# Rafae1130/qwen_inference_engine

Measured on AMD Instinct MI355X. Metric: decode tokens/s + prefill tok/s, Qwen2-7B bf16 batch=1, 1/2/4/8 MI355X, higher is better.
Workload: dtype bf16; 1 GPU; Qwen2-7B bf16 decode, batch=1, prompt=2048, gen=512; batch_per_gpu=1, batch=1, prompt=2048, gen=512, parallelism=single, graph=True, kv=contiguous

## Files before the change

__graft_entry__.py:

```python
import os
import subprocess
import sys

ROOT = os.path.dirname(os.path.abspath(__file__))


def build() -> None:
    jobs = str(min(16, os.cpu_count() or 8))
    subprocess.check_call(["make", "-s", "-j", jobs, "-C", os.path.join(ROOT, "qwen_inference_engine_amd", "csrc")])
    subprocess.check_call(["make", "-s", "-C", os.path.join(ROOT, "oracle")])
    if os.path.isdir("/root/reference/layers/src"):
        subprocess.check_call(["make", "-s", "-C", os.path.join(ROOT, "oracle"), "ref"])
    sys.path.insert(0, ROOT)
    import qwen_inference_engine_amd as q
    from qwen_inference_engine_amd import _lib
    _lib.load()


def smoke() -> None:
    sys.path.insert(0, ROOT)
    sys.path.insert(0, os.path.join(ROOT, "oracle"))
    import numpy as np
    import oracle as O
    import qwen_inference_engine_amd as q
# ... 19 lines not shown
```

include/qie/qie_ops.h:

```cpp
#ifndef QIE_OPS_H
#define QIE_OPS_H

#include "qie_types.h"

#ifdef __cplusplus
extern "C" {
#endif

#define QIE_ABI_VERSION 1

const char* qie_last_error(void);
int qie_abi_version(void);
int qie_device_count(int* count);

int qie_set_device(int device);
int qie_malloc(void** ptr, int64_t bytes);
int qie_free(void* ptr);
int qie_memcpy_h2d(void* dst, const void* src, int64_t bytes);
int qie_memcpy_d2h(void* dst, const void* src, int64_t bytes);
int qie_memset(void* ptr, int value, int64_t bytes);
int qie_synchronize(void);
int qie_stream_create(void** stream_out);
int qie_stream_synchronize(void* stream);
int qie_stream_destroy(void* stream);
// ... 52 lines not shown
                 int32_t layer, float eps, int32_t numerics, void* q_out, void* stream);

int64_t qie_attention_workspace_bytes(int64_t M, int32_t n_heads, int32_t head_dim,
                                      int32_t max_ctx);
int qie_attention(const void* q, int64_t M, const int32_t* pos, int32_t rows_per_seq,
                  const qie_kv_cache* cache, int32_t layer, int32_t n_heads, void* out,
                  void* ws, void* stream);

int64_t qie_attention_extend_workspace_bytes(int64_t M, int32_t n_heads, int32_t head_dim,
                                             int32_t max_ctx);
int32_t qie_attention_extend_split_tokens(int64_t M, int32_t max_ctx);
int qie_attention_extend(const void* q, int64_t M, const int32_t* pos, int32_t rows_per_seq,
                         const qie_kv_cache* cache, int32_t layer, int32_t n_heads, void* out,
                         void* ws, void* stream);

#define QIE_NUMERICS_MASK 0xff
#define QIE_ATTN_PREROPED 0x100
int64_t qie_attention_decode_workspace_bytes(int64_t B, int32_t n_heads, int32_t n_kv_heads,
                                             int32_t head_dim, int32_t max_ctx);
int qie_attention_decode(const void* qkv, int64_t B, const int32_t* pos, const void* q_norm,
                         const void* k_norm, const float* rope_cos, const float* rope_sin,
                         int32_t n_heads, const qie_kv_cache* cache, int32_t layer, float eps,
                         int32_t numerics, void* out, void* ws, void* stream);

int qie_debug_tr16_probe(int32_t* out_dev);

int qie_qknorm(void* x, int64_t rows, int64_t row_stride, int32_t n_heads, int32_t head_dim,
               const void* w, float eps, int32_t numerics, void* stream);
int qie_rope(void* x, int64_t rows, int64_t row_stride, int32_t n_heads, int32_t head_dim,
             const int32_t* pos, int32_t pos0, const float* rope_cos, const float* rope_sin,
// ... 57 lines not shown
```

qwen_inference_engine_amd/_lib.py:

```python
from __future__ import annotations

import ctypes as C
import os

_HERE = os.path.dirname(os.path.abspath(__file__))
LIB_PATH = os.environ.get("QIE_LIB") or os.path.join(_HERE, "lib", "libqie.so")

QIE_NUMERICS_REF = 0
QIE_NUMERICS_HF = 1
QIE_EPI_STORE = 0
QIE_EPI_RESIDUAL = 1
QIE_EPI_SWIGLU = 2
QIE_EPI_F32 = 3
QIE_LINEAR_FP8 = 1
QIE_LINEAR_TILE256 = 2
QIE_LINEAR_TILE128 = 4
QIE_LINEAR_STREAMK = 8
QIE_LINEAR_FP8_T16 = 16
QIE_LINEAR_ACT_FP8 = 32
QIE_ATTN_PREROPED = 0x100
QIE_VERIFY_MAX_ROWS = 16
QIE_SCORE_UNFUSED = 1
QIE_COMM_ID_BYTES = 128
QIE_COMM_PEER_HANDLE_BYTES = 128
# ... 70 lines not shown
    ("qie_stream_create", C.c_int, [C.POINTER(_P)]),
    ("qie_stream_synchronize", C.c_int, [_P]),
    ("qie_stream_destroy", C.c_int, [_P]),
    ("qie_rope_table_host", C.c_int, [_PF, _PF, _I32, _I32, _F, _I32]),
    ("qie_embedding", C.c_int, [_P, _P, _P, _I64, _I64, _P]),
    ("qie_rmsnorm", C.c_int, [_P, _P, _P, _I64, _I64, _F, _I32, _P]),
    ("qie_linear", C.c_int, [C.POINTER(LinearArgsC), _P]),
    ("qie_debug_linear_plan", C.c_int, [C.POINTER(LinearArgsC), C.c_char_p, C.c_int]),
    ("qie_qkv_post", C.c_int, [_P, _I64, _P, _I32, _P, _P, _P, _P, _I32, C.POINTER(KvCacheC),
                               _I32, _F, _I32, _P, _P]),
    ("qie_attention_workspace_bytes", C.c_int64, [_I64, _I32, _I32, _I32]),
    ("qie_attention", C.c_int, [_P, _I64, _P, _I32, C.POINTER(KvCacheC), _I32, _I32, _P, _P, _P]),
    ("qie_attention_extend_workspace_bytes", C.c_int64, [_I64, _I32, _I32, _I32]),
    ("qie_attention_extend_split_tokens", C.c_int32, [_I64, _I32]),
    ("qie_attention_extend", C.c_int, [_P, _I64, _P, _I32, C.POINTER(KvCacheC), _I32, _I32, _P, _P, _P]),
    ("qie_attention_decode_workspace_bytes", C.c_int64, [_I64, _I32, _I32, _I32, _I32]),
    ("qie_attention_decode", C.c_int, [_P, _I64, _P, _P, _P, _P, _P, _I32, C.POINTER(KvCacheC), _I32, _F, _I32,
                                       _P, _P, _P]),
    ("qie_debug_tr16_probe", C.c_int, [_P]),
    ("qie_qknorm", C.c_int, [_P, _I64, _I64, _I32, _I32, _P, _F, _I32, _P]),
    ("qie_rope", C.c_int, [_P, _I64, _I64, _I32, _I32, _P, _I32, _P, _P, _I32, _P]),
    ("qie_kv_write", C.c_int, [_P, _P, _I64, _I64, _I32, C.POINTER(KvCacheC), _I32, _I32, _P]),
    ("qie_kv_copy", C.c_int, [C.POINTER(KvCacheC), _I32, C.POINTER(KvCacheC), _I32, _I32, _I32, _P]),
    ("qie_silu", C.c_int, [_P, _I64, _P]),
    ("qie_mul", C.c_int, [_P, _P, _P, _I64, _P]),
    ("qie_memcpy_d2d", C.c_int, [_P, _P, _I64, _P]),
    ("qie_silu_mul", C.c_int, [_P, _P, _P, _I64, _P]),
    ("qie_residual_add", C.c_int, [_P, _P, _I64, _P]),
    ("qie_residual_add_f32", C.c_int, [_P, _P, _I64, _P]),
    ("qie_sample_workspace_bytes", C.c_int64, [_I64, _I64]),
# ... 113 lines not shown
```

qwen_inference_engine_amd/csrc/attn_mfma_tile.hpp:

```cpp
#pragma once
#include "attn_decode.hpp"

#include <type_traits>

namespace qie {

template <int HD, bool PG, int NW, bool SPLIT>
__device__ __forceinline__ void attn_mfma_walk(const uint16_t* kb, const uint16_t* vb, const KvMap& km, const int seq,
                                               const int kmax, const int k0, const int nkt,
                                               const bf16x8_t (&qf)[2][HD / 32], const int (&qpos)[2],
                                               const int (&gpos)[2], const int (&gmin)[2], f32x4_t (&oacc)[2][HD / 16],
                                               float (&m_run)[2], float (&l_run)[2]) {
    constexpr int KT = 64;
    constexpr int CPR = HD / 8;
    constexpr int KSTEPS = HD / 32;
    constexpr int DT = HD / 16;
    constexpr int QG = 2;
    extern __shared__ __attribute__((aligned(16))) unsigned char smem[];
    uint16_t* Ks = reinterpret_cast<uint16_t*>(smem);
    uint16_t* Vs = reinterpret_cast<uint16_t*>(smem + 2 * KT * HD * 2);
    auto vswz = [](int r) { return 2 * (r & (CPR / 2 - 1)); };

    const int tid = threadIdx.x, lane = tid & 63, wave = __builtin_amdgcn_readfirstlane(tid >> 6);
    const int fr = lane & 15, g = lane >> 4;
// ... 57 lines not shown
#pragma unroll
            for (int q = 0; q < QG; q++) {
                if (!ON[q]) continue;
                float (&sv)[4][4] = pv[q];
                float mt = -INFINITY;
                if (kt * KT + KT - 1 <= gmin[q]) {
#pragma unroll
                    for (int t = 0; t < 4; t++)
#pragma unroll
                        for (int r = 0; r < 4; r++) {
                            const float sc = sacc[q][t][r] * sl2;
                            sv[t][r] = sc;
                            mt = fmaxf(mt, sc);
                        }
                } else {
#pragma unroll
                    for (int t = 0; t < 4; t++)
#pragma unroll
                        for (int r = 0; r < 4; r++) {
                            const int key = kt * KT + t * 16 + g * 4 + r;
                            const float sc = key <= qpos[q] ? sacc[q][t][r] * sl2 : -INFINITY;
                            sv[t][r] = sc;
                            mt = fmaxf(mt, sc);
                        }
                }
                mt = xor32_max(xor16_max(mt));
                const float m_new = fmaxf(m_run[q], mt);
                const float m_use = SPLIT && m_new == -INFINITY ? 0.f : m_new;
                const float alpha = __builtin_amdgcn_exp2f(m_run[q] - m_use);
                float ls = 0.f;
#pragma unroll
                for (int t = 0; t < 4; t++)
#pragma unroll
                    for (int r = 0; r < 4; r++) {
                        const float e = __builtin_amdgcn_exp2f(sv[t][r] - m_use);
                        sv[t][r] = e;
// ... 99 lines not shown
```

qwen_inference_engine_amd/csrc/engine.hip:

```cpp
#include "qie_common.hpp"
#include "linear_plan.hpp"
#include "../../include/qie/qie_engine.h"
#include "qie_index.hpp"
#include "qie_comm.hpp"
#include "verify.hpp"
#include "row_bufs.hpp"
#include "page_pool.hpp"

#include <chrono>
#include <cstring>
#include <fstream>
#include <functional>
#include <vector>

namespace qie {
bool dec8_applies(const qie_linear_args* a);
int dec8_reserve(hipStream_t st);
bool persist_supported(const qie_model_spec& s, int B, int tp, bool fp8, bool paged, int ncu, const char** why);
size_t persist_attn_table_bytes(int n_layers);
int persist_attn_table(const qie_model_spec& s, const qie_layer_weights* h_layers, const void* qkv_scratch,
                       const int32_t* pos, const float* rope_cos, const float* rope_sin, const qie_kv_cache* cache,
                       void* dec_ws, void* d_attp, hipStream_t st);
int persist_decode_launch(const qie_model_spec& s, const qie_layer_weights* d_layers, const void* d_attp,
                          uint16_t* x_res, unsigned long long* granules, const unsigned* epoch, unsigned* err,
// ... 567 lines not shown

static int enqueue_layer_decode(qie_batch* b, int l) {
    qie_engine* e = b->e;
    const LayerPath p = decode_path(e);
    const qie_layer_weights& L = p.layers[l];
    const LayerRows r = layer_rows(b->dec, b->B, 1);
    QIE_TRY(run_proj(b, qkv_args(e, L, p.flags, r), p.in, r, decode_qkv_extras(b)));
    QIE_TRY(attend_decode(b, l, r.att));
    QIE_TRY(run_row_proj(b, o_args(e, L, p.flags, r), p.in, r));
    QIE_TRY(dbg_snap(b, 2 * l + 1));
    QIE_TRY(run_proj(b, gate_up_args(e, L, p.flags, r), p.in, r));
    QIE_TRY(run_row_proj(b, down_args(e, L, p.flags, r), p.in, r));
    return dbg_snap(b, 2 * l + 2);
}

using AttentionFn = decltype(&qie_attention);
static int enqueue_layer_rows(qie_batch* b, int l, const LayerRows& r, const LayerPath& p, const qie_kv_cache& cache,
                              AttentionFn attend, void* attn_ws) {
    qie_engine* e = b->e;
    const qie_model_spec& s = e->spec;
    const qie_layer_weights& L = p.layers[l];
    hipStream_t st = e->stream;
    QIE_TRY(run_proj(b, qkv_args(e, L, p.flags, r), p.in, r));
    QIE_TRY(qie_qkv_post(r.qkv, r.M, r.pos, r.rows_per_seq, L.q_norm, L.k_norm, e->rope_cos, e->rope_sin, e->sh.nq,
                         &cache, l, s.rms_eps, s.numerics, r.q, st));
    QIE_TRY(attend(r.q, r.M, r.pos, r.rows_per_seq, &cache, l, e->sh.nq, r.att, attn_ws, st));
    QIE_TRY(run_row_proj(b, o_args(e, L, p.flags, r), p.in, r));
    QIE_TRY(run_proj(b, gate_up_args(e, L, p.flags, r), p.in, r));
    return run_row_proj(b, down_args(e, L, p.flags, r), p.in, r);
}

static bool is_greedy(const qie_sampling* s) { return !s || s->top_k <= 1 || !(s->temperature > 0.f); }

__global__ void unshard_rows_kernel(const uint16_t* __restrict__ tmp, uint16_t* __restrict__ full, int tp, int M,
                                    int64_t Vl, int64_t V, int m0) {
    const int64_t n = (int64_t)tp * M * Vl;
    for (int64_t k = blockIdx.x * 256 + threadIdx.x; k < n; k += (int64_t)gridDim.x * 256) {
        const int64_t j = k % Vl, i = (k / Vl) % M, r = k / (Vl * M);
        full[(m0 + i) * V + r * Vl + j] = tmp[k];
    }
}
// ... 731 lines not shown
    }
    QIE_TRY(flush_table(b));
    const int64_t H = s.hidden;
    QIE_HIP(hipMemcpyAsync(b->pf.ids_in, ids, (size_t)n * 4, hipMemcpyHostToDevice, st));
    hipLaunchKernelGGL(iota_kernel, dim3((unsigned)((n + 255) / 256)), dim3(256), 0, st, b->pf.pos, (int)n, len, pos0);
    hipLaunchKernelGGL(copy_ids_kernel, dim3((len + 255) / 256, n_seqs), dim3(256), 0, st, b->pf.ids_in,
                       b->dec.hist + (int64_t)seq0 * b->max_ctx + pos0, len, (int64_t)b->max_ctx);
    QIE_TRY(qie_embedding(e->w.embed, b->pf.ids_in, b->pf.x, n, H, st));
    const qie_kv_cache cache = batch_cache(b, seq0);
    const LayerRows r = layer_rows(b->pf, n, len);
    const bool pf16 = e->fp8 && !e->layers_pf.empty() && (n >= 256 || (e->fp8_t16 && n > 16));
    LayerPath path{e->layers.data(), proj_flags(e), prefill_mx(e) ? InputForm::Fp8 : InputForm::Normed};
    if (pf16 && path.in == InputForm::Normed)
        path = LayerPath{e->layers_pf.data(), path.flags & ~(QIE_LINEAR_FP8 | QIE_LINEAR_FP8_T16), InputForm::Normed};
    for (int l = 0; l < s.n_layers; l++)
        QIE_TRY(enqueue_layer_rows(b, l, r, path, cache, append ? qie_attention_extend : qie_attention, b->pf_ws.p));
    for (int z = 0; z < n_seqs; z++) {
        hipLaunchKernelGGL(set_state_kernel, dim3(1), dim3(64), 0, st, seq0 + z, pos0 + len - 1, 0,
                           ids[(int64_t)z * len + len - 1], b->dec.pos, b->dec.step, b->dec.hist, b->max_ctx,
                           (const uint4*)e->w.embed, (uint4*)b->dec.x, (int64_t)H / 8, 0, rope_cur_args(b));
        QIE_LAUNCH_CHECK();
    }
    const uint16_t* last = b->pf.x + (int64_t)(len - 1) * H;
    if (n_seqs > 1) {
        QIE_HIP(hipMemcpy2DAsync(b->pf.xn, (size_t)H * 2, last, (size_t)len * H * 2, (size_t)H * 2, n_seqs,
                                 hipMemcpyDeviceToDevice, st));
        last = b->pf.xn;
    }
    QIE_TRY(enqueue_head(b, last, H, seq0, n_seqs, smp));
    for (int z = 0; z < n_seqs; z++) b->h_pos[seq0 + z] = pos0 + len;
    if (score) QIE_TRY(enqueue_score(b, seq0, len, *score));
// ... 358 lines not shown
    b->v = v;
    return 0;
}

static int enqueue_verify(qie_batch* b, int seq, int M, const qie_sampling* smp) {
    qie_engine* e = b->e;
    const qie_model_spec& s = e->spec;
    hipStream_t st = e->stream;
    const int64_t H8 = (int64_t)s.hidden / 8;
    VerifyRowsArgs ra{seq, M, b->v.draft, s.vocab, (const uint4*)e->w.embed, (const uint4*)b->dec.x, H8,
                      b->dec.pos, b->dec.step, (uint4*)b->v.x, b->v.pos, b->v.step};
    QIE_TRY(launch_verify_rows(ra, st));
    const qie_kv_cache cache = batch_cache(b, seq);
    const LayerRows r = layer_rows(b->v, M, M);
    for (int l = 0; l < s.n_layers; l++)
        QIE_TRY(enqueue_layer_rows(b, l, r, decode_path(e), cache, qie_attention_extend, b->v.attn_ws));
    QIE_TRY(enqueue_head_rows(b, b->v.x, s.hidden, M, smp, head_bufs(b->v, 0, b->e->sh.vocab)));
    const bool greedy = is_greedy(smp);
    VerifyCommitArgs ca{seq, M, greedy ? b->v.keys : nullptr, b->v.ids, b->v.draft, s.vocab, b->dec.pos, b->dec.step,
                        b->dec.hist, b->max_ctx, b->dec.ids, (const uint4*)e->w.embed, (uint4*)b->dec.x, H8,
                        rope_cur_args(b), b->v.logits, b->dec.logits, (int64_t)e->sh.vocab, b->v.res};
    return launch_verify_commit(ca, st);
}

static int launch_verify(qie_batch* b, int seq, int M, const qie_sampling* smp) {
    qie_engine* e = b->e;
    if (!e->opts.use_graph) return enqueue_verify(b, seq, M, smp);
    const bool greedy = is_greedy(smp);
    for (const auto& g : b->v_graphs)
        if (g.seq == seq && g.M == M && g.greedy == greedy && (greedy || same_sampling(g.smp, smp))) {
            QIE_HIP(hipGraphLaunch(g.exec, e->stream));
// ... 311 lines not shown
```

qwen_inference_engine_amd/csrc/k_attention.hip:

```cpp
#include "qie_common.hpp"
#include "../../include/qie/qie_ops.h"
#include "attn_mfma_tile.hpp"


#include <cstdlib>
#include <type_traits>

namespace qie {

struct AttnParams {
    const uint16_t* q;
    const int32_t* pos;
    int rows_per_seq;
    const uint16_t* kc;
    const uint16_t* vc;
    KvMap km;
    int layer, nkv, nq, max_ctx;
    int nsplit;
    float* part_o;
    float* part_ml;
    uint16_t* out;
};

template <int HD, bool PG>
__global__ __launch_bounds__(256) void attn_split_kernel(AttnParams a) {
    constexpr int LPT = HD / 8;
// ... 2 lines not shown
    __shared__ float sm_m[4][kMaxGroup], sm_l[4][kMaxGroup];

    const int64_t m = blockIdx.y;
    const int g = blockIdx.x / a.nsplit, s = blockIdx.x % a.nsplit;
    const int G = a.nq / a.nkv;
    const int lane = threadIdx.x & 63, wave = threadIdx.x >> 6;
    const int sub = lane / LPT, dl = lane % LPT;
    const int ctx = a.pos[m] + 1;
    int chunk = (ctx + a.nsplit - 1) / a.nsplit;
    chunk = (chunk + 4 * TPW - 1) / (4 * TPW) * (4 * TPW);
    const int t0 = s * chunk;
    const int t1 = min(ctx, t0 + chunk);
    const int64_t seq = m / a.rows_per_seq;

    float qf[kMaxGroup][8];
    const uint16_t* qrow = a.q + m * (int64_t)a.nq * HD + (int64_t)g * G * HD + dl * 8;
#pragma unroll
    for (int gi = 0; gi < kMaxGroup; gi++) {
        if (gi < G) {
            uint4 v = *reinterpret_cast<const uint4*>(qrow + gi * HD);
            uint32_t w[4] = {v.x, v.y, v.z, v.w};
#pragma unroll
            for (int j = 0; j < 4; j++) {
                qf[gi][2 * j] = bf_lo(w[j]);
                qf[gi][2 * j + 1] = bf_hi(w[j]);
            }
        } else {
#pragma unroll
            for (int j = 0; j < 8; j++) qf[gi][j] = 0.f;
        }
    }
    float mr[kMaxGroup], lr[kMaxGroup], o[kMaxGroup][8];
#pragma unroll
    for (int gi = 0; gi < kMaxGroup; gi++) {
        mr[gi] = -INFINITY;
// ... 88 lines not shown
        if (a.nsplit == 1) {
            a.out[m * (int64_t)a.nq * HD + (int64_t)h * HD + d] = f2bf(ov / l);
        } else {
            const int64_t pi = (m * a.nq + h) * (int64_t)a.nsplit + s;
            a.part_o[pi * HD + d] = ov;
            if (d == 0) {
                a.part_ml[pi * 2] = mn;
                a.part_ml[pi * 2 + 1] = l;
            }
        }
    }
}


struct PrefillAttnParams {
    const uint16_t* q;
    const int32_t* pos;
    int rows_per_seq;
    const uint16_t* kc;
    const uint16_t* vc;
    KvMap km;
    int layer, nkv, nq;
    uint16_t* out;
    int full_tiles;
};


template <int HD, bool PG, int NW>
__global__ __launch_bounds__(64 * NW, 8 / NW) void attn_prefill_mfma2_kernel(PrefillAttnParams a) {
    constexpr int KT = 64;
    constexpr int KSTEPS = HD / 32;
// ... 15 lines not shown
    bool gact[QG];
    gact[0] = j < npair;
    gact[1] = j < npair && grp[1] != j;
    const int kmax = a.pos[row0 + min(16 * (ngr - 1 - (int)blockIdx.x * NW) + 15, R - 1)];
    const int nkt = kmax / KT + 1;

    int qpos[QG], gpos[QG], gmin[QG];
    bf16x8_t qf[QG][KSTEPS];
#pragma unroll
    for (int q = 0; q < QG; q++) {
        const int gq = gact[q] ? grp[q] : 0;
        const int qrow = min(16 * gq + fr, R - 1);
        qpos[q] = a.pos[row0 + qrow];
        gpos[q] = __builtin_amdgcn_readfirstlane(gact[q] ? a.pos[row0 + min(16 * gq + 15, R - 1)] : -1);
        gmin[q] = __builtin_amdgcn_readfirstlane(a.full_tiles ? a.pos[row0 + min(16 * gq, R - 1)] : -1);
        const uint16_t* qp = a.q + (row0 + qrow) * (int64_t)a.nq * HD + (int64_t)h * HD;
#pragma unroll
        for (int ks = 0; ks < KSTEPS; ks++) qf[q][ks] = *reinterpret_cast<const bf16x8_t*>(qp + ks * 32 + g * 8);
    }

    f32x4_t oacc[QG][DT];
    float m_run[QG], l_run[QG];
    attn_mfma_walk<HD, PG, NW, false>(kb, vb, a.km, seq, kmax, 0, nkt, qf, qpos, gpos, gmin, oacc, m_run, l_run);
#pragma unroll
    for (int q = 0; q < QG; q++) {
        if (!gact[q]) continue;
        float lr[4];
#pragma unroll
        for (int r = 0; r < 4; r++) lr[r] = __shfl(l_run[q], g * 4 + r, 64);
#pragma unroll
        for (int r = 0; r < 4; r++) {
            const int row = 16 * grp[q] + g * 4 + r;
            if (row >= R) continue;
// ... 84 lines not shown
                           out, ws);
}

}

using namespace qie;

extern "C" {

int64_t qie_attention_workspace_bytes(int64_t M, int32_t n_heads, int32_t head_dim, int32_t max_ctx) {
    const int ns = attn_nsplit(M, max_ctx);
    if (ns == 1) return 0;
    return M * n_heads * (int64_t)ns * (head_dim + 2) * 4;
}

int qie_attention(const void* q, int64_t M, const int32_t* pos, int32_t rows_per_seq,
                  const qie_kv_cache* cache, int32_t layer, int32_t n_heads, void* out, void* ws,
                  void* stream) {
    QIE_REQUIRE(q && pos && cache && cache->k && cache->v && out && M >= 0 && rows_per_seq > 0,
                "qie_attention: bad arguments");
    QIE_REQUIRE(cache->head_dim == 64 || cache->head_dim == 128,
                "qie_attention: head_dim must be 64 or 128 (got %d)", cache->head_dim);
    QIE_REQUIRE(n_heads % cache->n_kv_heads == 0 && n_heads / cache->n_kv_heads <= kMaxGroup,
                "qie_attention: n_heads/n_kv_heads must be an integer <= %d", kMaxGroup);
    QIE_REQUIRE(layer >= 0 && layer < cache->n_layers, "qie_attention: bad layer");
    if (M == 0) return 0;
    if (rows_per_seq >= 32 && M % rows_per_seq == 0) {
        PrefillAttnParams pa;
        pa.q = (const uint16_t*)q;
        pa.pos = pos;
        pa.rows_per_seq = rows_per_seq;
        pa.kc = (const uint16_t*)cache->k;
        pa.vc = (const uint16_t*)cache->v;
        QIE_TRY(kv_map_make(cache, &pa.km, "qie_attention"));
        pa.layer = layer;
        pa.nkv = cache->n_kv_heads;
        pa.nq = n_heads;
        pa.out = (uint16_t*)out;
        pa.full_tiles = dev_env("QIE_ATTN_PF_FULL", 1);
        const size_t shm = (size_t)2 * 2 * 64 * cache->head_dim * 2;
        const bool pg = pa.km.table != nullptr;
        const int npair = ((rows_per_seq + 15) / 16 + 1) / 2;
        const int nw = dev_env("QIE_ATTN_PF_NW", 8) == 4 ? 4 : 8;
        dim3 g2((unsigned)((npair + nw - 1) / nw), (unsigned)n_heads, (unsigned)(M / rows_per_seq));
        auto k2 = nw == 8 ? (cache->head_dim == 128 ? (pg ? attn_prefill_mfma2_kernel<128, true, 8> : attn_prefill_mfma2_kernel<128, false, 8>)
                                                    : (pg ? attn_prefill_mfma2_kernel<64, true, 8> : attn_prefill_mfma2_kernel<64, false, 8>))
                          : (cache->head_dim == 128 ? (pg ? attn_prefill_mfma2_kernel<128, true, 4> : attn_prefill_mfma2_kernel<128, false, 4>)
                                                    : (pg ? attn_prefill_mfma2_kernel<64, true, 4> : attn_prefill_mfma2_kernel<64, false, 4>));
        hipLaunchKernelGGL(k2, g2, dim3(64 * nw), shm, (hipStream_t)stream, pa);
        QIE_LAUNCH_CHECK();
        return 0;
    }
    AttnParams a;
    a.q = (const uint16_t*)q;
    a.pos = pos;
    a.rows_per_seq = rows_per_seq;
    a.kc = (const uint16_t*)cache->k;
    a.vc = (const uint16_t*)cache->v;
    QIE_TRY(kv_map_make(cache, &a.km, "qie_attention"));
    a.layer = layer;
    a.nkv = cache->n_kv_heads;
    a.nq = n_heads;
    a.max_ctx = cache->max_ctx;
    a.nsplit = attn_nsplit(M, cache->max_ctx);
    const int64_t part = M * n_heads * (int64_t)a.nsplit;
    a.part_o = (float*)ws;
    a.part_ml = ws ? (float*)ws + part * cache->head_dim : nullptr;
    a.out = (uint16_t*)out;
    QIE_REQUIRE(a.nsplit == 1 || ws, "qie_attention: workspace required");
    hipStream_t st = (hipStream_t)stream;
    dim3 grid((unsigned)(a.nkv * a.nsplit), (unsigned)M);
    const bool pg = a.km.table != nullptr;
    auto k = cache->head_dim == 128 ? (pg ? attn_split_kernel<128, true> : attn_split_kernel<128, false>)
                                    : (pg ? attn_split_kernel<64, true> : attn_split_kernel<64, false>);
    hipLaunchKernelGGL(k, grid, dim3(256), 0, st, a);
    QIE_LAUNCH_CHECK();
    if (a.nsplit > 1) {
        launch_attn_combine<false>(cache->head_dim, M, n_heads, a.nsplit, a.part_o, a.part_ml, a.out, st);
        QIE_LAUNCH_CHECK();
    }
    return 0;
}

int qie_debug_tr16_probe(int32_t* out_dev) {
    QIE_REQUIRE(out_dev, "qie_debug_tr16_probe: null");
    hipLaunchKernelGGL(tr16_probe_kernel, dim3(1), dim3(64), 0, nullptr, out_dev);
    QIE_LAUNCH_CHECK();
    return 0;
}

int64_t qie_attention_decode_workspace_bytes(int64_t B, int32_t n_heads, int32_t n_kv_heads, int32_t head_dim,
                                             int32_t max_ctx) {
    const int64_t ns = std::min<int64_t>(kDecMaxSplits, (max_ctx + 63) / 64);
    const int64_t cnt = ((B * n_kv_heads * 4 + 255) / 256) * 256;
    return cnt + B * n_heads * ns * (head_dim + 2) * 4;
}
// ... 37 lines not shown
```

qwen_inference_engine_amd/csrc/k_attn_extend.hip:

```cpp
#include "qie_common.hpp"
#include "../../include/qie/qie_ops.h"
#include "attn_mfma_tile.hpp"

namespace qie {

constexpr int kExtSplitLong = 512;
constexpr int kExtSplitShort = 256;
constexpr int kExtShortRows = 32;
constexpr int kExtMaxSplits = 64;
constexpr int kExtBlockRows = 128;

static void extend_split(int64_t M, int32_t max_ctx, int* len, int* count) {
    int L = M <= kExtShortRows ? kExtSplitShort : kExtSplitLong;
    int n = (max_ctx + L - 1) / L;
    while (n > kExtMaxSplits) {
        L *= 2;
        n = (max_ctx + L - 1) / L;
    }
    *len = L;
    *count = n < 1 ? 1 : n;
}

struct ExtendAttnParams {
    const uint16_t* q;
    const int32_t* pos;
    int rows_per_seq;
    int64_t M;
    const uint16_t* kc;
    const uint16_t* vc;
    KvMap km;
    int layer, nkv, nq;
    int nsplit, split_len;
    float* part_o;
    float* part_ml;
    uint16_t* out;
};

template <int HD, bool PG>
__global__ __launch_bounds__(256, 2) void attn_extend_kernel(ExtendAttnParams a) {
// ... 35 lines not shown
    const uint16_t* vb = a.vc + head_off;

    const int grp[QG] = {wave, NGB - 1 - wave};
    bool gact[QG];
    int qpos[QG], gpos[QG], gmin[QG];
    bf16x8_t qf[QG][KSTEPS];
#pragma unroll
    for (int q = 0; q < QG; q++) {
        gact[q] = f0 + 16 * grp[q] < RG;
        const int fb = gact[q] ? f0 + 16 * grp[q] : f0;
        const int f = min(fb + fr, RG - 1);
        const int t = f / G, hq = f - t * G;
        qpos[q] = a.pos[row0 + t];
        gpos[q] = __builtin_amdgcn_readfirstlane(gact[q] ? a.pos[row0 + min(fb + 15, RG - 1) / G] : -1);
        gmin[q] = __builtin_amdgcn_readfirstlane(a.pos[row0 + fb / G]);
        const uint16_t* qp = a.q + (row0 + t) * (int64_t)a.nq * HD + (int64_t)(kvh * G + hq) * HD;
#pragma unroll
        for (int ks = 0; ks < KSTEPS; ks++) qf[q][ks] = *reinterpret_cast<const bf16x8_t*>(qp + ks * 32 + g * 8);
    }

    f32x4_t oacc[QG][DT];
    float m_run[QG], l_run[QG];
    attn_mfma_walk<HD, PG, NW, true>(kb, vb, a.km, seq, kmax, k0, nkt, qf, qpos, gpos, gmin, oacc, m_run, l_run);

#pragma unroll
    for (int q = 0; q < QG; q++) {
        if (!gact[q]) continue;
        const int fb = f0 + 16 * grp[q];
        if (a.nsplit == 1) {
            float lr[4];
#pragma unroll
            for (int r = 0; r < 4; r++) lr[r] = __shfl(l_run[q], g * 4 + r, 64);
#pragma unroll
// ... 29 lines not shown
extern "C" {

int32_t qie_attention_extend_split_tokens(int64_t M, int32_t max_ctx) {
    int len, count;
    extend_split(M, max_ctx, &len, &count);
    return len;
}

int64_t qie_attention_extend_workspace_bytes(int64_t M, int32_t n_heads, int32_t head_dim, int32_t max_ctx) {
    int len, count;
    extend_split(M, max_ctx, &len, &count);
    if (count == 1) return 0;
    return M * n_heads * (int64_t)count * (head_dim + 2) * 4;
}

int qie_attention_extend(const void* q, int64_t M, const int32_t* pos, int32_t rows_per_seq,
                         const qie_kv_cache* cache, int32_t layer, int32_t n_heads, void* out, void* ws,
                         void* stream) {
    QIE_REQUIRE(q && pos && cache && cache->k && cache->v && out && M >= 0 && rows_per_seq > 0 && n_heads > 0,
                "qie_attention_extend: bad arguments");
    QIE_REQUIRE(cache->head_dim == 64 || cache->head_dim == 128,
                "qie_attention_extend: head_dim must be 64 or 128 (got %d)", cache->head_dim);
    QIE_REQUIRE(cache->n_kv_heads > 0 && n_heads % cache->n_kv_heads == 0 &&
                    n_heads / cache->n_kv_heads <= kMaxGroup,
                "qie_attention_extend: n_heads/n_kv_heads must be an integer <= %d", kMaxGroup);
    QIE_REQUIRE(layer >= 0 && layer < cache->n_layers, "qie_attention_extend: bad layer");
    if (M == 0) return 0;
    ExtendAttnParams a;
    a.q = (const uint16_t*)q;
    a.pos = pos;
    a.rows_per_seq = rows_per_seq;
    a.M = M;
    a.kc = (const uint16_t*)cache->k;
    a.vc = (const uint16_t*)cache->v;
    QIE_TRY(kv_map_make(cache, &a.km, "qie_attention_extend"));
    a.layer = layer;
    a.nkv = cache->n_kv_heads;
    a.nq = n_heads;
    extend_split(M, cache->max_ctx, &a.split_len, &a.nsplit);
    QIE_REQUIRE(a.nsplit == 1 || ws, "qie_attention_extend: workspace required");
    const int64_t part = M * n_heads * (int64_t)a.nsplit;
    a.part_o = (float*)ws;
    a.part_ml = ws ? (float*)ws + part * cache->head_dim : nullptr;
    a.out = (uint16_t*)out;
// ... 5 lines not shown
    hipStream_t st = (hipStream_t)stream;
    const size_t shm = (size_t)2 * 2 * 64 * cache->head_dim * 2;
    const bool pg = a.km.table != nullptr;
    dim3 grid((unsigned)nblk, (unsigned)a.nsplit, (unsigned)(n_seqs * a.nkv));
    auto k = cache->head_dim == 128 ? (pg ? attn_extend_kernel<128, true> : attn_extend_kernel<128, false>)
                                    : (pg ? attn_extend_kernel<64, true> : attn_extend_kernel<64, false>);
    hipLaunchKernelGGL(k, grid, dim3(256), shm, st, a);
    QIE_LAUNCH_CHECK();
    if (a.nsplit > 1) {
        launch_attn_combine<true>(cache->head_dim, M, n_heads, a.nsplit, a.part_o, a.part_ml, a.out, st);
        QIE_LAUNCH_CHECK();
    }
    return 0;
}

}
```

qwen_inference_engine_amd/csrc/k_misc.hip:

```cpp
#include "qie_common.hpp"
#include "launch_util.hpp"
#include "../../include/qie/qie_ops.h"

#include <cmath>
#include <cstdarg>
#include <cstring>
#include <map>
#include <mutex>
#include <tuple>
#include <vector>

#ifdef _OPENMP
#include <omp.h>
#endif

namespace qie {

static thread_local std::string g_last_error;

void set_error(const std::string& msg) { g_last_error = msg; }

int fail(int code, const char* fmt, ...) {
    char buf[1024];
    va_list ap;
// ... 196 lines not shown
            float x0 = active ? bf2f((uint16_t)(raw[b] & 0xffffu)) : 0.f;
            float x1 = active ? bf2f((uint16_t)(raw[b] >> 16)) : 0.f;
            if (rope && nw) {
                float ss = wave_sum(x0 * x0 + x1 * x1);
                float rms = sqrtf((ss / (float)hd) + a.eps);
                if (HF) {
                    float inv = 1.0f / rms;
                    x0 = rbf(bf2f(nw[i0]) * rbf(x0 * inv));
                    x1 = rbf(bf2f(nw[i1]) * rbf(x1 * inv));
                } else {
                    x0 = rbf((x0 / rms) * bf2f(nw[i0]));
                    x1 = rbf((x1 / rms) * bf2f(nw[i1]));
                }
            }
            float y0 = x0, y1 = x1;
            if (rope) {
                if (HF) {
                    y0 = rbf(rbf(x0 * c) + rbf(-x1 * s));
                    y1 = rbf(rbf(x1 * c) + rbf(x0 * s));
                } else {
                    y0 = x0 * c - x1 * s;
                    y1 = x1 * c + x0 * s;
                }
            }
            if (active) {
                if (HF) {
                    dst[i0] = f2bf(y0);
                    dst[i1] = f2bf(y1);
                } else {
                    reinterpret_cast<uint32_t*>(dst)[lane] = pack2(y0, y1);
                }
            }
        }
    }
}

struct HeadOpArgs {
    uint16_t* x;
    int64_t row_stride;
    int nheads, hd;
    const uint16_t* w;
    float eps;
    const float* cs;
    const float* sn;
    const int32_t* pos;
    int pos0;
    int numerics;
    int rope;
};
// ... 404 lines not shown
    a.kc = (uint16_t*)cache->k;
    a.vc = (uint16_t*)cache->v;
    QIE_TRY(kv_map_make(cache, &a.km, "qie_qkv_post"));
    a.layer = layer;
    a.eps = eps;
    a.numerics = numerics;
    a.q_out = (uint16_t*)q_out;
    const bool hf = numerics == QIE_NUMERICS_HF;
    auto fn = a.km.table ? (hf ? qkv_post_kernel<true, true> : qkv_post_kernel<true, false>)
                         : (hf ? qkv_post_kernel<false, true> : qkv_post_kernel<false, false>);
    hipLaunchKernelGGL(fn, dim3((unsigned)M), dim3(256), 0, (hipStream_t)stream, a);
    QIE_LAUNCH_CHECK();
    return 0;
}

int qie_memcpy_d2d(void* dst, const void* src, int64_t bytes, void* stream) {
    QIE_REQUIRE(dst && src && bytes >= 0, "qie_memcpy_d2d: bad arguments");
    if (bytes == 0) return 0;
    QIE_HIP(hipMemcpyAsync(dst, src, (size_t)bytes, hipMemcpyDeviceToDevice, (hipStream_t)stream));
    return 0;
}

int qie_qknorm(void* x, int64_t rows, int64_t row_stride, int32_t n_heads, int32_t head_dim, const void* w,
               float eps, int32_t numerics, void* stream) {
    QIE_REQUIRE(w, "qie_qknorm: null weight");
    HeadOpArgs a{};
    a.x = (uint16_t*)x; a.row_stride = row_stride; a.nheads = n_heads; a.hd = head_dim;
    a.w = (const uint16_t*)w; a.eps = eps; a.numerics = numerics; a.rope = 0;
    QIE_REQUIRE(a.x && rows >= 0 && n_heads > 0 && head_dim > 0 && head_dim % 2 == 0 && head_dim <= 128 &&
                    row_stride >= (int64_t)n_heads * head_dim,
// ... 308 lines not shown
```

Measured before the change: 368.1 tokens/s.

## Fuse Q RoPE into prefill attention and write K/V with a lightweight kernel

```diff
diff --git a/__graft_entry__.py b/__graft_entry__.py
--- a/__graft_entry__.py
+++ b/__graft_entry__.py
@@ -8,6 +8,8 @@
 def build() -> None:
     jobs = str(min(16, os.cpu_count() or 8))
     subprocess.check_call(["make", "-s", "-j", jobs, "-C", os.path.join(ROOT, "qwen_inference_engine_amd", "csrc")])
+    subprocess.check_call(["make", "-s", "-j", jobs, "-C", os.path.join(ROOT, "qwen_inference_engine_amd", "csrc"),
+                           "DEV=1"])
     subprocess.check_call(["make", "-s", "-C", os.path.join(ROOT, "oracle")])
     if os.path.isdir("/root/reference/layers/src"):
         subprocess.check_call(["make", "-s", "-C", os.path.join(ROOT, "oracle"), "ref"])
diff --git a/include/qie/qie_ops.h b/include/qie/qie_ops.h
--- a/include/qie/qie_ops.h
+++ b/include/qie/qie_ops.h
@@ -90,6 +90,18 @@
                          const qie_kv_cache* cache, int32_t layer, int32_t n_heads, void* out,
                          void* ws, void* stream);
 
+int qie_kv_post(const void* qkv, int64_t ld, int64_t M, const int32_t* pos, int32_t rows_per_seq,
+                const float* rope_cos, const float* rope_sin, int32_t n_heads,
+                const qie_kv_cache* cache, int32_t layer, int32_t numerics, void* stream);
+int qie_attention_qkv(const void* qkv, int64_t ld, int64_t M, const int32_t* pos,
+                      int32_t rows_per_seq, const float* rope_cos, const float* rope_sin,
+                      int32_t numerics, const qie_kv_cache* cache, int32_t layer, int32_t n_heads,
+                      void* out, void* ws, void* stream);
+int qie_attention_extend_qkv(const void* qkv, int64_t ld, int64_t M, const int32_t* pos,
+                             int32_t rows_per_seq, const float* rope_cos, const float* rope_sin,
+                             int32_t numerics, const qie_kv_cache* cache, int32_t layer,
+                             int32_t n_heads, void* out, void* ws, void* stream);
+
 #define QIE_NUMERICS_MASK 0xff
 #define QIE_ATTN_PREROPED 0x100
 int64_t qie_attention_decode_workspace_bytes(int64_t B, int32_t n_heads, int32_t n_kv_heads,
diff --git a/qwen_inference_engine_amd/_lib.py b/qwen_inference_engine_amd/_lib.py
--- a/qwen_inference_engine_amd/_lib.py
+++ b/qwen_inference_engine_amd/_lib.py
@@ -108,6 +108,11 @@
     ("qie_attention_extend_workspace_bytes", C.c_int64, [_I64, _I32, _I32, _I32]),
     ("qie_attention_extend_split_tokens", C.c_int32, [_I64, _I32]),
     ("qie_attention_extend", C.c_int, [_P, _I64, _P, _I32, C.POINTER(KvCacheC), _I32, _I32, _P, _P, _P]),
+    ("qie_kv_post", C.c_int, [_P, _I64, _I64, _P, _I32, _P, _P, _I32, C.POINTER(KvCacheC), _I32, _I32, _P]),
+    ("qie_attention_qkv", C.c_int, [_P, _I64, _I64, _P, _I32, _P, _P, _I32, C.POINTER(KvCacheC), _I32, _I32,
+                                    _P, _P, _P]),
+    ("qie_attention_extend_qkv", C.c_int, [_P, _I64, _I64, _P, _I32, _P, _P, _I32, C.POINTER(KvCacheC), _I32, _I32,
+                                           _P, _P, _P]),
     ("qie_attention_decode_workspace_bytes", C.c_int64, [_I64, _I32, _I32, _I32, _I32]),
     ("qie_attention_decode", C.c_int, [_P, _I64, _P, _P, _P, _P, _P, _I32, C.POINTER(KvCacheC), _I32, _F, _I32,
                                        _P, _P, _P]),
diff --git a/qwen_inference_engine_amd/csrc/attn_mfma_tile.hpp b/qwen_inference_engine_amd/csrc/attn_mfma_tile.hpp
--- a/qwen_inference_engine_amd/csrc/attn_mfma_tile.hpp
+++ b/qwen_inference_engine_amd/csrc/attn_mfma_tile.hpp
@@ -95,12 +95,12 @@
                             mt = fmaxf(mt, sc);
                         }
                 } else {
+                    const int rel = qpos[q] - kt * KT - g * 4;
 #pragma unroll
                     for (int t = 0; t < 4; t++)
 #pragma unroll
                         for (int r = 0; r < 4; r++) {
-                            const int key = kt * KT + t * 16 + g * 4 + r;
-                            const float sc = key <= qpos[q] ? sacc[q][t][r] * sl2 : -INFINITY;
+                            const float sc = t * 16 + r <= rel ? sacc[q][t][r] * sl2 : -INFINITY;
                             sv[t][r] = sc;
                             mt = fmaxf(mt, sc);
                         }
diff --git a/qwen_inference_engine_amd/csrc/engine.hip b/qwen_inference_engine_amd/csrc/engine.hip
--- a/qwen_inference_engine_amd/csrc/engine.hip
+++ b/qwen_inference_engine_amd/csrc/engine.hip
@@ -605,17 +605,27 @@
     return dbg_snap(b, 2 * l + 2);
 }
 
-using AttentionFn = decltype(&qie_attention);
+enum class RowAttention { FromZero, Extend };
 static int enqueue_layer_rows(qie_batch* b, int l, const LayerRows& r, const LayerPath& p, const qie_kv_cache& cache,
-                              AttentionFn attend, void* attn_ws) {
+                              RowAttention form, void* attn_ws, bool q_prologue) {
     qie_engine* e = b->e;
     const qie_model_spec& s = e->spec;
     const qie_layer_weights& L = p.layers[l];
     hipStream_t st = e->stream;
     QIE_TRY(run_proj(b, qkv_args(e, L, p.flags, r), p.in, r));
-    QIE_TRY(qie_qkv_post(r.qkv, r.M, r.pos, r.rows_per_seq, L.q_norm, L.k_norm, e->rope_cos, e->rope_sin, e->sh.nq,
-                         &cache, l, s.rms_eps, s.numerics, r.q, st));
-    QIE_TRY(attend(r.q, r.M, r.pos, r.rows_per_seq, &cache, l, e->sh.nq, r.att, attn_ws, st));
+    if (q_prologue && !s.qk_norm && dev_env("QIE_ATTN_QPROLOGUE", 1) != 0) {
+        const auto attend = form == RowAttention::Extend ? qie_attention_extend_qkv : qie_attention_qkv;
+        const int64_t ld = (int64_t)(e->sh.nq + 2 * cache.n_kv_heads) * cache.head_dim;
+        QIE_TRY(qie_kv_post(r.qkv, ld, r.M, r.pos, r.rows_per_seq, e->rope_cos, e->rope_sin, e->sh.nq, &cache, l,
+                            s.numerics, st));
+        QIE_TRY(attend(r.qkv, ld, r.M, r.pos, r.rows_per_seq, e->rope_cos, e->rope_sin, s.numerics, &cache, l,
+                       e->sh.nq, r.att, attn_ws, st));
+    } else {
+        const auto attend = form == RowAttention::Extend ? qie_attention_extend : qie_attention;
+        QIE_TRY(qie_qkv_post(r.qkv, r.M, r.pos, r.rows_per_seq, L.q_norm, L.k_norm, e->rope_cos, e->rope_sin,
+                             e->sh.nq, &cache, l, s.rms_eps, s.numerics, r.q, st));
+        QIE_TRY(attend(r.q, r.M, r.pos, r.rows_per_seq, &cache, l, e->sh.nq, r.att, attn_ws, st));
+    }
     QIE_TRY(run_row_proj(b, o_args(e, L, p.flags, r), p.in, r));
     QIE_TRY(run_proj(b, gate_up_args(e, L, p.flags, r), p.in, r));
     return run_row_proj(b, down_args(e, L, p.flags, r), p.in, r);
@@ -1377,7 +1387,8 @@
     if (pf16 && path.in == InputForm::Normed)
         path = LayerPath{e->layers_pf.data(), path.flags & ~(QIE_LINEAR_FP8 | QIE_LINEAR_FP8_T16), InputForm::Normed};
     for (int l = 0; l < s.n_layers; l++)
-        QIE_TRY(enqueue_layer_rows(b, l, r, path, cache, append ? qie_attention_extend : qie_attention, b->pf_ws.p));
+        QIE_TRY(enqueue_layer_rows(b, l, r, path, cache, append ? RowAttention::Extend : RowAttention::FromZero,
+                                   b->pf_ws.p, true));
     for (int z = 0; z < n_seqs; z++) {
         hipLaunchKernelGGL(set_state_kernel, dim3(1), dim3(64), 0, st, seq0 + z, pos0 + len - 1, 0,
                            ids[(int64_t)z * len + len - 1], b->dec.pos, b->dec.step, b->dec.hist, b->max_ctx,
@@ -1766,7 +1777,7 @@
     const qie_kv_cache cache = batch_cache(b, seq);
     const LayerRows r = layer_rows(b->v, M, M);
     for (int l = 0; l < s.n_layers; l++)
-        QIE_TRY(enqueue_layer_rows(b, l, r, decode_path(e), cache, qie_attention_extend, b->v.attn_ws));
+        QIE_TRY(enqueue_layer_rows(b, l, r, decode_path(e), cache, RowAttention::Extend, b->v.attn_ws, false));
     QIE_TRY(enqueue_head_rows(b, b->v.x, s.hidden, M, smp, head_bufs(b->v, 0, b->e->sh.vocab)));
     const bool greedy = is_greedy(smp);
     VerifyCommitArgs ca{seq, M, greedy ? b->v.keys : nullptr, b->v.ids, b->v.draft, s.vocab, b->dec.pos, b->dec.step,
diff --git a/qwen_inference_engine_amd/csrc/k_attention.hip b/qwen_inference_engine_amd/csrc/k_attention.hip
--- a/qwen_inference_engine_amd/csrc/k_attention.hip
+++ b/qwen_inference_engine_amd/csrc/k_attention.hip
@@ -1,6 +1,7 @@
 #include "qie_common.hpp"
 #include "../../include/qie/qie_ops.h"
 #include "attn_mfma_tile.hpp"
+#include "rope_rotate.hpp"
 
 
 #include <cstdlib>
@@ -9,7 +10,7 @@
 namespace qie {
 
 struct AttnParams {
-    const uint16_t* q;
+    QSource qs;
     const int32_t* pos;
     int rows_per_seq;
     const uint16_t* kc;
@@ -42,11 +43,11 @@
     const int64_t seq = m / a.rows_per_seq;
 
     float qf[kMaxGroup][8];
-    const uint16_t* qrow = a.q + m * (int64_t)a.nq * HD + (int64_t)g * G * HD + dl * 8;
+    const uint16_t* qrow = a.qs.q + m * a.qs.ld + (int64_t)g * G * HD;
 #pragma unroll
     for (int gi = 0; gi < kMaxGroup; gi++) {
         if (gi < G) {
-            uint4 v = *reinterpret_cast<const uint4*>(qrow + gi * HD);
+            uint4 v = load_q8(a.qs, qrow + gi * HD, dl * 8, HD, ctx - 1);
             uint32_t w[4] = {v.x, v.y, v.z, v.w};
 #pragma unroll
             for (int j = 0; j < 4; j++) {
@@ -165,7 +166,7 @@
 
 
 struct PrefillAttnParams {
-    const uint16_t* q;
+    QSource qs;
     const int32_t* pos;
     int rows_per_seq;
     const uint16_t* kc;
@@ -211,9 +212,10 @@
         qpos[q] = a.pos[row0 + qrow];
         gpos[q] = __builtin_amdgcn_readfirstlane(gact[q] ? a.pos[row0 + min(16 * gq + 15, R - 1)] : -1);
         gmin[q] = __builtin_amdgcn_readfirstlane(a.full_tiles ? a.pos[row0 + min(16 * gq, R - 1)] : -1);
-        const uint16_t* qp = a.q + (row0 + qrow) * (int64_t)a.nq * HD + (int64_t)h * HD;
-#pragma unroll
-        for (int ks = 0; ks < KSTEPS; ks++) qf[q][ks] = *reinterpret_cast<const bf16x8_t*>(qp + ks * 32 + g * 8);
+        const uint16_t* qp = a.qs.q + (row0 + qrow) * a.qs.ld + (int64_t)h * HD;
+#pragma unroll
+        for (int ks = 0; ks < KSTEPS; ks++)
+            qf[q][ks] = __builtin_bit_cast(bf16x8_t, load_q8(a.qs, qp, ks * 32 + g * 8, HD, qpos[q]));
     }
 
     f32x4_t oacc[QG][DT];
@@ -328,10 +330,10 @@
     return M * n_heads * (int64_t)ns * (head_dim + 2) * 4;
 }
 
-int qie_attention(const void* q, int64_t M, const int32_t* pos, int32_t rows_per_seq,
-                  const qie_kv_cache* cache, int32_t layer, int32_t n_heads, void* out, void* ws,
-                  void* stream) {
-    QIE_REQUIRE(q && pos && cache && cache->k && cache->v && out && M >= 0 && rows_per_seq > 0,
+static int attention_rows(const QSource& qs, int64_t M, const int32_t* pos, int32_t rows_per_seq,
+                          const qie_kv_cache* cache, int32_t layer, int32_t n_heads, void* out, void* ws,
+                          void* stream) {
+    QIE_REQUIRE(qs.q && pos && cache && cache->k && cache->v && out && M >= 0 && rows_per_seq > 0,
                 "qie_attention: bad arguments");
     QIE_REQUIRE(cache->head_dim == 64 || cache->head_dim == 128,
                 "qie_attention: head_dim must be 64 or 128 (got %d)", cache->head_dim);
@@ -341,7 +343,7 @@
     if (M == 0) return 0;
     if (rows_per_seq >= 32 && M % rows_per_seq == 0) {
         PrefillAttnParams pa;
-        pa.q = (const uint16_t*)q;
+        pa.qs = qs;
         pa.pos = pos;
         pa.rows_per_seq = rows_per_seq;
         pa.kc = (const uint16_t*)cache->k;
@@ -366,7 +368,7 @@
         return 0;
     }
     AttnParams a;
-    a.q = (const uint16_t*)q;
+    a.qs = qs;
     a.pos = pos;
     a.rows_per_seq = rows_per_seq;
     a.kc = (const uint16_t*)cache->k;
@@ -394,6 +396,21 @@
         QIE_LAUNCH_CHECK();
     }
     return 0;
+}
+
+int qie_attention(const void* q, int64_t M, const int32_t* pos, int32_t rows_per_seq,
+                  const qie_kv_cache* cache, int32_t layer, int32_t n_heads, void* out, void* ws,
+                  void* stream) {
+    const QSource qs{(const uint16_t*)q, cache ? (int64_t)n_heads * cache->head_dim : 0, nullptr, nullptr, 0};
+    return attention_rows(qs, M, pos, rows_per_seq, cache, layer, n_heads, out, ws, stream);
+}
+
+int qie_attention_qkv(const void* qkv, int64_t ld, int64_t M, const int32_t* pos, int32_t rows_per_seq,
+                      const float* rope_cos, const float* rope_sin, int32_t numerics, const qie_kv_cache* cache,
+                      int32_t layer, int32_t n_heads, void* out, void* ws, void* stream) {
+    QSource qs;
+    QIE_TRY(q_source_make(&qs, qkv, ld, rope_cos, rope_sin, numerics, cache, n_heads, "qie_attention_qkv"));
+    return attention_rows(qs, M, pos, rows_per_seq, cache, layer, n_heads, out, ws, stream);
 }
 
 int qie_debug_tr16_probe(int32_t* out_dev) {
diff --git a/qwen_inference_engine_amd/csrc/k_attn_extend.hip b/qwen_inference_engine_amd/csrc/k_attn_extend.hip
--- a/qwen_inference_engine_amd/csrc/k_attn_extend.hip
+++ b/qwen_inference_engine_amd/csrc/k_attn_extend.hip
@@ -1,6 +1,7 @@
 #include "qie_common.hpp"
 #include "../../include/qie/qie_ops.h"
 #include "attn_mfma_tile.hpp"
+#include "rope_rotate.hpp"
 
 namespace qie {
 
@@ -22,7 +23,7 @@
 }
 
 struct ExtendAttnParams {
-    const uint16_t* q;
+    QSource qs;
     const int32_t* pos;
     int rows_per_seq;
     int64_t M;
@@ -88,9 +89,10 @@
         qpos[q] = a.pos[row0 + t];
         gpos[q] = __builtin_amdgcn_readfirstlane(gact[q] ? a.pos[row0 + min(fb + 15, RG - 1) / G] : -1);
         gmin[q] = __builtin_amdgcn_readfirstlane(a.pos[row0 + fb / G]);
-        const uint16_t* qp = a.q + (row0 + t) * (int64_t)a.nq * HD + (int64_t)(kvh * G + hq) * HD;
-#pragma unroll
-        for (int ks = 0; ks < KSTEPS; ks++) qf[q][ks] = *reinterpret_cast<const bf16x8_t*>(qp + ks * 32 + g * 8);
+        const uint16_t* qp = a.qs.q + (row0 + t) * a.qs.ld + (int64_t)(kvh * G + hq) * HD;
+#pragma unroll
+        for (int ks = 0; ks < KSTEPS; ks++)
+            qf[q][ks] = __builtin_bit_cast(bf16x8_t, load_q8(a.qs, qp, ks * 32 + g * 8, HD, qpos[q]));
     }
 
     f32x4_t oacc[QG][DT];
@@ -150,10 +152,10 @@
     return M * n_heads * (int64_t)count * (head_dim + 2) * 4;
 }
 
-int qie_attention_extend(const void* q, int64_t M, const int32_t* pos, int32_t rows_per_seq,
-                         const qie_kv_cache* cache, int32_t layer, int32_t n_heads, void* out, void* ws,
-                         void* stream) {
-    QIE_REQUIRE(q && pos && cache && cache->k && cache->v && out && M >= 0 && rows_per_seq > 0 && n_heads > 0,
+static int attention_extend_rows(const QSource& qs, int64_t M, const int32_t* pos, int32_t rows_per_seq,
+                                 const qie_kv_cache* cache, int32_t layer, int32_t n_heads, void* out, void* ws,
+                                 void* stream) {
+    QIE_REQUIRE(qs.q && pos && cache && cache->k && cache->v && out && M >= 0 && rows_per_seq > 0 && n_heads > 0,
                 "qie_attention_extend: bad arguments");
     QIE_REQUIRE(cache->head_dim == 64 || cache->head_dim == 128,
                 "qie_attention_extend: head_dim must be 64 or 128 (got %d)", cache->head_dim);
@@ -163,7 +165,7 @@
     QIE_REQUIRE(layer >= 0 && layer < cache->n_layers, "qie_attention_extend: bad layer");
     if (M == 0) return 0;
     ExtendAttnParams a;
-    a.q = (const uint16_t*)q;
+    a.qs = qs;
     a.pos = pos;
     a.rows_per_seq = rows_per_seq;
     a.M = M;
@@ -199,4 +201,20 @@
     return 0;
 }
 
-}
+int qie_attention_extend(const void* q, int64_t M, const int32_t* pos, int32_t rows_per_seq,
+                         const qie_kv_cache* cache, int32_t layer, int32_t n_heads, void* out, void* ws,
+                         void* stream) {
+    const QSource qs{(const uint16_t*)q, cache ? (int64_t)n_heads * cache->head_dim : 0, nullptr, nullptr, 0};
+    return attention_extend_rows(qs, M, pos, rows_per_seq, cache, layer, n_heads, out, ws, stream);
+}
+
+int qie_attention_extend_qkv(const void* qkv, int64_t ld, int64_t M, const int32_t* pos, int32_t rows_per_seq,
+                             const float* rope_cos, const float* rope_sin, int32_t numerics,
+                             const qie_kv_cache* cache, int32_t layer, int32_t n_heads, void* out, void* ws,
+                             void* stream) {
+    QSource qs;
+    QIE_TRY(q_source_make(&qs, qkv, ld, rope_cos, rope_sin, numerics, cache, n_heads, "qie_attention_extend_qkv"));
+    return attention_extend_rows(qs, M, pos, rows_per_seq, cache, layer, n_heads, out, ws, stream);
+}
+
+}
diff --git a/qwen_inference_engine_amd/csrc/k_misc.hip b/qwen_inference_engine_amd/csrc/k_misc.hip
--- a/qwen_inference_engine_amd/csrc/k_misc.hip
+++ b/qwen_inference_engine_amd/csrc/k_misc.hip
@@ -1,5 +1,6 @@
 #include "qie_common.hpp"
 #include "launch_util.hpp"
+#include "rope_rotate.hpp"
 #include "../../include/qie/qie_ops.h"
 
 #include <cmath>
@@ -234,15 +235,7 @@
                 }
             }
             float y0 = x0, y1 = x1;
-            if (rope) {
-                if (HF) {
-                    y0 = rbf(rbf(x0 * c) + rbf(-x1 * s));
-                    y1 = rbf(rbf(x1 * c) + rbf(x0 * s));
-                } else {
-                    y0 = x0 * c - x1 * s;
-                    y1 = x1 * c + x0 * s;
-                }
-            }
+            if (rope) rope_rotate<HF>(x0, x1, c, s, y0, y1);
             if (active) {
                 if (HF) {
                     dst[i0] = f2bf(y0);
@@ -253,6 +246,40 @@
             }
         }
     }
+}
+
+struct KvPostArgs {
+    const uint16_t* qkv;
+    int64_t ld;
+    const int32_t* pos;
+    int rows_per_seq;
+    uint32_t total;
+    const float* cs;
+    const float* sn;
+    int nq, nkv, hd;
+    uint16_t* kc;
+    uint16_t* vc;
+    KvMap km;
+    int layer;
+};
+
+template <bool PG, bool HF>
+__global__ __launch_bounds__(256) void kv_post_kernel(KvPostArgs a) {
+    const uint32_t cph = a.hd / 8;
+    const uint32_t cpr = 2 * a.nkv * cph;
+    const uint32_t idx = blockIdx.x * 256 + threadIdx.x;
+    if (idx >= a.total) return;
+    const uint32_t m = idx / cpr, c = idx - m * cpr;
+    const int hh = c / cph, d0 = (c - hh * cph) * 8;
+    const bool isk = hh < a.nkv;
+    const int g = isk ? hh : hh - a.nkv;
+    const int p = a.pos[m];
+    const int64_t seq = m / a.rows_per_seq;
+    const uint16_t* src = a.qkv + m * a.ld + (int64_t)(a.nq + hh) * a.hd;
+    uint16_t* dst = (isk ? a.kc : a.vc) + kv_run_off(a.km, (int64_t)a.layer * a.nkv + g, a.hd) +
+                    kv_tok<PG>(a.km, seq, p, a.hd) + d0;
+    *reinterpret_cast<uint4*>(dst) =
+        isk ? rope_chunk8<HF>(src, d0, a.hd, a.cs, a.sn, p) : *reinterpret_cast<const uint4*>(src + d0);
 }
 
 struct HeadOpArgs {
@@ -687,6 +714,45 @@
     return 0;
 }
 
+int qie_kv_post(const void* qkv, int64_t ld, int64_t M, const int32_t* pos, int32_t rows_per_seq,
+                const float* rope_cos, const float* rope_sin, int32_t n_heads, const qie_kv_cache* cache,
+                int32_t layer, int32_t numerics, void* stream) {
+    QIE_REQUIRE(qkv && pos && cache && cache->k && cache->v && rope_cos && rope_sin && M >= 0 && rows_per_seq > 0 &&
+                    n_heads > 0 && cache->n_kv_heads > 0 && layer >= 0 && layer < cache->n_layers,
+                "qie_kv_post: bad arguments");
+    const int hd = cache->head_dim, nkv = cache->n_kv_heads;
+    QIE_REQUIRE(hd > 0 && hd % 16 == 0, "qie_kv_post: head_dim must be a multiple of 16 (got %d)", hd);
+    QIE_REQUIRE(ld >= (int64_t)(n_heads + 2 * nkv) * hd && ld % 8 == 0, "qie_kv_post: bad row stride %lld", (long long)ld);
+    QIE_REQUIRE((((uintptr_t)qkv | (uintptr_t)cache->k | (uintptr_t)cache->v | (uintptr_t)rope_cos | (uintptr_t)rope_sin) & 15) == 0 &&
+                    cache->seq_stride % 8 == 0,
+                "qie_kv_post: rows, tables and cache must be 16-byte aligned");
+    QIE_REQUIRE(numerics == QIE_NUMERICS_REF || numerics == QIE_NUMERICS_HF, "qie_kv_post: bad numerics %d", numerics);
+    if (M == 0) return 0;
+    const int64_t total = M * 2 * nkv * (hd / 8);
+    QIE_REQUIRE(total < ((int64_t)1 << 31), "qie_kv_post: %lld rows are too many for one launch", (long long)M);
+    KvPostArgs a;
+    a.qkv = (const uint16_t*)qkv;
+    a.ld = ld;
+    a.pos = pos;
+    a.rows_per_seq = rows_per_seq;
+    a.total = (uint32_t)total;
+    a.cs = rope_cos;
+    a.sn = rope_sin;
+    a.nq = n_heads;
+    a.nkv = nkv;
+    a.hd = hd;
+    a.kc = (uint16_t*)cache->k;
+    a.vc = (uint16_t*)cache->v;
+    QIE_TRY(kv_map_make(cache, &a.km, "qie_kv_post"));
+    a.layer = layer;
+    const bool hf = numerics == QIE_NUMERICS_HF;
+    auto fn = a.km.table ? (hf ? kv_post_kernel<true, true> : kv_post_kernel<true, false>)
+                         : (hf ? kv_post_kernel<false, true> : kv_post_kernel<false, false>);
+    hipLaunchKernelGGL(fn, dim3((unsigned)((total + 255) / 256)), dim3(256), 0, (hipStream_t)stream, a);
+    QIE_LAUNCH_CHECK();
+    return 0;
+}
+
 int qie_memcpy_d2d(void* dst, const void* src, int64_t bytes, void* stream) {
     QIE_REQUIRE(dst && src && bytes >= 0, "qie_memcpy_d2d: bad arguments");
     if (bytes == 0) return 0;
diff --git a/qwen_inference_engine_amd/csrc/rope_rotate.hpp b/qwen_inference_engine_amd/csrc/rope_rotate.hpp
--- /dev/null
+++ b/qwen_inference_engine_amd/csrc/rope_rotate.hpp
@@ -0,0 +1,85 @@
+#pragma once
+#include "qie_common.hpp"
+#include "../../include/qie/qie_ops.h"
+
+namespace qie {
+
+template <bool HF>
+__device__ __forceinline__ void rope_rotate(float x0, float x1, float c, float s, float& y0, float& y1) {
+#pragma clang fp contract(off)
+    if (HF) {
+        y0 = rbf(rbf(x0 * c) + rbf(-x1 * s));
+        y1 = rbf(rbf(x1 * c) + rbf(x0 * s));
+    } else {
+        y0 = x0 * c - x1 * s;
+        y1 = x1 * c + x0 * s;
+    }
+}
+
+template <bool HF>
+__device__ __forceinline__ uint4 rope_chunk8(const uint16_t* head, int d0, int hd, const float* cs, const float* sn,
+                                             int64_t p) {
+    const int half = hd / 2;
+    const uint4 own = *reinterpret_cast<const uint4*>(head + d0);
+    const uint32_t w[4] = {own.x, own.y, own.z, own.w};
+    uint32_t o[4];
+    if (HF) {
+        const bool lo = d0 < half;
+        const uint4 oth = *reinterpret_cast<const uint4*>(head + (lo ? d0 + half : d0 - half));
+        const uint32_t v[4] = {oth.x, oth.y, oth.z, oth.w};
+        const float* cp = cs + p * half + (lo ? d0 : d0 - half);
+        const float* sp = sn + p * half + (lo ? d0 : d0 - half);
+        const float4 c4[2] = {reinterpret_cast<const float4*>(cp)[0], reinterpret_cast<const float4*>(cp)[1]};
+        const float4 s4[2] = {reinterpret_cast<const float4*>(sp)[0], reinterpret_cast<const float4*>(sp)[1]};
+        const float c[8] = {c4[0].x, c4[0].y, c4[0].z, c4[0].w, c4[1].x, c4[1].y, c4[1].z, c4[1].w};
+        const float s[8] = {s4[0].x, s4[0].y, s4[0].z, s4[0].w, s4[1].x, s4[1].y, s4[1].z, s4[1].w};
+        float y[8];
+#pragma unroll
+        for (int j = 0; j < 8; j++) {
+            const float xo = (j & 1) ? bf_hi(w[j >> 1]) : bf_lo(w[j >> 1]);
+            const float xp = (j & 1) ? bf_hi(v[j >> 1]) : bf_lo(v[j >> 1]);
+            float y0, y1;
+            rope_rotate<true>(lo ? xo : xp, lo ? xp : xo, c[j], s[j], y0, y1);
+            y[j] = lo ? y0 : y1;
+        }
+#pragma unroll
+        for (int j = 0; j < 4; j++) o[j] = pack2(y[2 * j], y[2 * j + 1]);
+    } else {
+        const float4 c4 = *reinterpret_cast<const float4*>(cs + p * half + d0 / 2);
+        const float4 s4 = *reinterpret_cast<const float4*>(sn + p * half + d0 / 2);
+        const float c[4] = {c4.x, c4.y, c4.z, c4.w}, s[4] = {s4.x, s4.y, s4.z, s4.w};
+#pragma unroll
+        for (int j = 0; j < 4; j++) {
+            float y0, y1;
+            rope_rotate<false>(bf_lo(w[j]), bf_hi(w[j]), c[j], s[j], y0, y1);
+            o[j] = pack2(y0, y1);
+        }
+    }
+    return make_uint4(o[0], o[1], o[2], o[3]);
+}
+
+struct QSource {
+    const uint16_t* q;
+    int64_t ld;
+    const float* cs;
+    const float* sn;
+    int hf;
+};
+
+inline int q_source_make(QSource* s, const void* qkv, int64_t ld, const float* rope_cos, const float* rope_sin,
+                         int32_t numerics, const qie_kv_cache* cache, int32_t n_heads, const char* who) {
+    QIE_REQUIRE(qkv && rope_cos && rope_sin && cache && n_heads > 0, "%s: bad arguments", who);
+    QIE_REQUIRE(ld >= (int64_t)n_heads * cache->head_dim && ld % 8 == 0, "%s: bad row stride %lld", who, (long long)ld);
+    QIE_REQUIRE((((uintptr_t)qkv | (uintptr_t)rope_cos | (uintptr_t)rope_sin) & 15) == 0,
+                "%s: rows and RoPE tables must be 16-byte aligned", who);
+    QIE_REQUIRE(numerics == QIE_NUMERICS_REF || numerics == QIE_NUMERICS_HF, "%s: bad numerics %d", who, numerics);
+    *s = QSource{(const uint16_t*)qkv, ld, rope_cos, rope_sin, numerics == QIE_NUMERICS_HF};
+    return 0;
+}
+
+__device__ __forceinline__ uint4 load_q8(const QSource& s, const uint16_t* head, int d0, int hd, int p) {
+    if (s.cs == nullptr) return *reinterpret_cast<const uint4*>(head + d0);
+    return s.hf ? rope_chunk8<true>(head, d0, hd, s.cs, s.sn, p) : rope_chunk8<false>(head, d0, hd, s.cs, s.sn, p);
+}
+
+}
```

New measurement: 368.9 tokens/s (median of 6 runs). About the same (+0.2%).
